# JonasFrey96/Visual-Odom-Pipeline

Hardware: AMD Instinct MI355X
Metric: frames/sec @1241x376, 2000 KLT pts, 10-frame BA window (higher is better)
Workload: dtype u8/i32 (KLT, Shi-Tomasi) + f64 (DLT, BA); 1 GPU; kitti_shaped_1241x376_2000pts_ba10; sequences_per_gpu=256, batched_contexts_per_gpu=1, distinct_image_sequences=8, tracked_points=jittered grid (SURVEY 8d's fallback), launch=plain, solves_stopped_by_cap=0, solves_cut_and_rerun=0

## Files before the change

include/vo_mi355x.h:

```cpp
#ifndef VO_MI355X_H
#define VO_MI355X_H

#include <stdint.h>

#ifdef __cplusplus
extern "C" {
#endif

#define VO_ABI_VERSION 4

enum {
  VO_OK = 0,
  VO_E_INVALID = -1,
  VO_E_HIP = -2,
  VO_E_NOMEM = -3,
  VO_E_STATE = -4,
  VO_E_CAPACITY = -5,
  VO_E_NUMERIC = -6
};

typedef struct vo_ctx vo_ctx;


typedef struct {
// ... 78 lines not shown
  int32_t pad;
} vo_ess_stats;

typedef struct {
  float   x, y;
  float   size;
  float   angle;
  float   response;
  int32_t octave;
} vo_sift_kp;

int32_t vo_abi_version(void);
int32_t vo_device_count(int32_t* n);
int32_t vo_ctx_create(int32_t device, int32_t width, int32_t height, int32_t max_pts,
                      int32_t max_level, int32_t win, vo_ctx** out);
int32_t vo_ctx_create_batched(int32_t device, int32_t width, int32_t height, int32_t max_pts,
                              int32_t max_level, int32_t win, int32_t batch, vo_ctx** out);
int32_t vo_ctx_destroy(vo_ctx* ctx);
const char* vo_last_error(const vo_ctx* ctx);
int32_t vo_sync(vo_ctx* ctx);

int32_t vo_frame_push(vo_ctx* ctx, const uint8_t* img, int32_t stride);
int32_t vo_set_prefilter(vo_ctx* ctx, int32_t d, double sigma_color, double sigma_space);
int32_t vo_set_undistort(vo_ctx* ctx, const double K[4], const double* dist, int32_t n_dist, const double* newK);
int32_t vo_clear_undistort(vo_ctx* ctx);
int32_t vo_get_undistort(vo_ctx* ctx, int32_t* on, double K[4], double dist[8], double newK[4]);
int32_t vo_undistort(vo_ctx* ctx, const uint8_t* img, int32_t stride, uint8_t* out);
int32_t vo_undistort_map_read(vo_ctx* ctx, int16_t* sxy, uint16_t* frac, uint8_t* outside);
int32_t vo_seq_upload(vo_ctx* ctx, const uint8_t* frames, int32_t n_frames);
int32_t vo_frame_push_resident(vo_ctx* ctx, int32_t frame_index);
int32_t vo_pyramid_level_size(vo_ctx* ctx, int32_t level, int32_t* w, int32_t* h);
int32_t vo_pyramid_read(vo_ctx* ctx, int32_t which, int32_t level, uint8_t* img_out, int16_t* deriv_out);
int32_t vo_pyramid_read_seq(vo_ctx* ctx, int32_t seq, int32_t which, int32_t level, uint8_t* img_out, int16_t* deriv_out);

int32_t vo_klt_default_params(vo_klt_params* p);
int32_t vo_klt_track(vo_ctx* ctx, const float* p0, int32_t n, const vo_klt_params* prm,
                     float* p1, uint8_t* status, float* err, int32_t* iters);
int32_t vo_points_upload(vo_ctx* ctx, const float* p, int32_t n);
int32_t vo_points_download(vo_ctx* ctx, float* p, uint8_t* status, float* err, int32_t* iters, int32_t n);
int32_t vo_klt_track_resident(vo_ctx* ctx, int32_t n, const vo_klt_params* prm);

int32_t vo_klt_track_fb(vo_ctx* ctx, const float* p0, int32_t n, const vo_klt_params* prm, float* p1, uint8_t* status, float* err,
                        float* p0r, float* fb_err, int32_t* iters);
int32_t vo_set_fb_check(vo_ctx* ctx, float max_err);
int32_t vo_get_fb_check(vo_ctx* ctx, float* max_err);
int32_t vo_fb_read(vo_ctx* ctx, uint8_t* ok, float* fb_err, int32_t n);

enum { VO_KLT_PREDICT_OFF = 0, VO_KLT_PREDICT_CONST_VELOCITY = 1 };
int32_t vo_klt_track_init(vo_ctx* ctx, const float* p0, const float* guess, int32_t n, const vo_klt_params* prm,
                          float* p1, uint8_t* status, float* err, int32_t* iters);
int32_t vo_klt_track_fb_init(vo_ctx* ctx, const float* p0, const float* guess, int32_t n, const vo_klt_params* prm, float* p1, uint8_t* status,
                             float* err, float* p0r, float* fb_err, int32_t* iters);
int32_t vo_set_klt_predict(vo_ctx* ctx, int32_t mode);
int32_t vo_get_klt_predict(vo_ctx* ctx, int32_t* mode);
int32_t vo_klt_guess_read(vo_ctx* ctx, float* guess, int32_t n);

int32_t vo_st_default_params(vo_st_params* p);
int32_t vo_shi_tomasi(vo_ctx* ctx, const float* cur_pts, int32_t n_cur, int32_t mask_radius,
                      const uint8_t* mask, const vo_st_params* prm, float* out_pts, int32_t* n_out);
int32_t vo_shi_tomasi_resident(vo_ctx* ctx, int32_t n_cur, int32_t mask_radius,
                               const vo_st_params* prm);
int32_t vo_shi_tomasi_fetch(vo_ctx* ctx, float* out_pts, int32_t* n_out);
int32_t vo_shi_tomasi_read(vo_ctx* ctx, float* eig_out, uint8_t* mask_out, int32_t* n_candidates);

typedef struct { int32_t win_x, win_y, zero_x, zero_y, max_count, _pad; double epsilon; } vo_subpix_params;
int32_t vo_subpix_default_params(vo_subpix_params* p);
// ... 177 lines not shown
```

visual-odom-pipeline_amd/csrc/vo_frame.hip:

```cpp
#include "vo_internal.h"

#include <stdlib.h>
#include <string.h>

#include <new>

__device__ __forceinline__ int d_reflect101(int p, int len) {
  if (len == 1) return 0;
  while (p < 0 || p >= len) p = (p < 0) ? -p : 2 * (len - 1) - p;
  return p;
}

struct bil_args {
  int maxk;
  signed char dx[49], dy[49];
  float sw[49];
};

__global__ void __launch_bounds__(256) k_pad_level0_bilateral(const uint8_t* __restrict__ raw, size_t raw_seq_stride,
                                                              const int32_t* __restrict__ frame_idx, int w, int h,
                                                              uint8_t* __restrict__ dst, size_t dst_seq_stride, int pitch,
                                                              int ph, bil_args A, const float* __restrict__ color_w) {
  __shared__ float s_cw[256];
  s_cw[threadIdx.x] = color_w[threadIdx.x];
  __syncthreads();
  const int X = blockIdx.x * blockDim.x + threadIdx.x;
  const int Y = blockIdx.y;
  if (X >= w + 2 * VO_PAD || Y >= ph) return;
  raw += (size_t)blockIdx.z * raw_seq_stride;
  dst += (size_t)blockIdx.z * dst_seq_stride;
  if (frame_idx) raw += (size_t)(*frame_idx) * w * h;
  const int x = d_reflect101(X - VO_PAD, w), y = d_reflect101(Y - VO_PAD, h);
  const int val0 = raw[(size_t)y * w + x];
  float sum = 0.f, wsum = 0.f;
  for (int k = 0; k < A.maxk; k++) {
    const int val = raw[(size_t)d_reflect101(y + A.dy[k], h) * w + d_reflect101(x + A.dx[k], w)];
    const int ad = val > val0 ? val - val0 : val0 - val;
    const float wt = A.sw[k] * s_cw[ad];
    sum += (float)val * wt;
    wsum += wt;
  }
  dst[(size_t)Y * pitch + X] = (uint8_t)(int)__builtin_rintf(sum / wsum);
}
// ... 15 lines not shown

__global__ void __launch_bounds__(256) k_pad_level0(const uint8_t* __restrict__ raw, size_t raw_seq_stride,
                                                    const int32_t* __restrict__ frame_idx, int w, int h,
                                                    uint8_t* __restrict__ dst, size_t dst_seq_stride, int pitch, int ph, int remap) {
  int blk, bseq;
  vo_xcd_assign(blockIdx.z * gridDim.x + blockIdx.x, gridDim.x, remap, blk, bseq);
  const int gpr = (w + 2 * VO_PAD + 15) / 16;
  const unsigned gid = (unsigned)blk * blockDim.x + threadIdx.x;
  const int g_lo = VO_PAD / 16, g_hi = max(g_lo, min(gpr, (w + VO_PAD - 16 >= 0 ? (w + VO_PAD - 16) / 16 + 1 : 0)));
  int Y, G;
  const bool interior = vo_split_index(gid, ph, gpr, g_lo, g_hi, Y, G);
  const int X = G * 16;
  if (Y >= ph) return;
  raw += (size_t)bseq * raw_seq_stride;
  dst += (size_t)bseq * dst_seq_stride;
  if (frame_idx) raw += (size_t)(*frame_idx) * w * h;
  const int y = d_reflect101(Y - VO_PAD, h);
  const uint8_t* row = raw + (size_t)y * w;
  uint32_t v[4];
  if (interior) {
    __builtin_memcpy(v, row + (X - VO_PAD), 16);
  } else {
#pragma unroll
    for (int q = 0; q < 4; q++) {
      v[q] = 0;
#pragma unroll
      for (int k = 0; k < 4; k++) v[q] |= (uint32_t)row[d_reflect101(X + 4 * q + k - VO_PAD, w)] << (8 * k);
    }
  }
  uint4 pk; pk.x = v[0]; pk.y = v[1]; pk.z = v[2]; pk.w = v[3];
  *reinterpret_cast<uint4*>(dst + (size_t)Y * pitch + X) = pk;
}

__device__ __forceinline__ int d_byte(uint32_t v, int k) { return (int)((v >> (8 * k)) & 0xFFu); }

__global__ void __launch_bounds__(256) k_scharr_pyrdown(const uint8_t* __restrict__ src, size_t src_seq_px, int w, int h, int pitch,
                                                        int16_t* __restrict__ der, int nb_scharr,
                                                        uint8_t* __restrict__ dst, size_t dst_seq_px, int dw, int dh, int dpitch, int remap) {
  int bx, bseq;
  vo_xcd_assign(blockIdx.y * gridDim.x + blockIdx.x, gridDim.x, remap, bx, bseq);
  src += (size_t)bseq * src_seq_px;
  if (bx < nb_scharr) {
    constexpr int SR = 4;
    const int gpr = (w + 3) / 4;
    const unsigned gid = (unsigned)bx * 256u + threadIdx.x;
    const int ys = (int)(gid / (unsigned)gpr);
    const int x0 = (int)(gid - (unsigned)ys * (unsigned)gpr) * 4;
    const int y0 = ys * SR;
    if (y0 >= h) return;
    typedef unsigned short u16x2 __attribute__((ext_vector_type(2)));
    typedef short s16x2 __attribute__((ext_vector_type(2)));
    auto load_row = [&](int yy, u16x2 (&a)[3]) {
      const uint32_t* q = reinterpret_cast<const uint32_t*>(src + (size_t)(yy + VO_PAD) * pitch + (x0 + VO_PAD));
      const uint32_t L = q[-1], M = q[0], R = q[1];
      a[0] = __builtin_bit_cast(u16x2, __builtin_amdgcn_perm(M, L, 0x0c040c03u));
      a[1] = __builtin_bit_cast(u16x2, __builtin_amdgcn_perm(0u, M, 0x0c020c01u));
      a[2] = __builtin_bit_cast(u16x2, __builtin_amdgcn_perm(R, M, 0x0c040c03u));
    };
    u16x2 rows[SR + 2][3];
#pragma unroll
    for (int r = 0; r < SR + 2; r++) load_row(min(y0 - 1 + r, h), rows[r]);
#pragma unroll
    for (int r = 0; r < SR; r++) {
      const int y = y0 + r;
      if (y >= h) break;
      s16x2 cs[3], dv[3];
#pragma unroll
      for (int c = 0; c < 3; c++) {
        cs[c] = __builtin_bit_cast(s16x2, (u16x2)((rows[r][c] + rows[r + 2][c]) * (unsigned short)12 + rows[r + 1][c] * (unsigned short)40));
        dv[c] = __builtin_bit_cast(s16x2, (u16x2)(rows[r + 2][c] - rows[r][c]));
      }
      const uint32_t ix01 = __builtin_bit_cast(uint32_t, (s16x2)(cs[1] - cs[0]));
      const uint32_t ix23 = __builtin_bit_cast(uint32_t, (s16x2)(cs[2] - cs[1]));
      const s16x2 w_lo = {12, 40}, w_hi = {40, 12}, w_0 = {12, 0}, w_1 = {0, 12};
      const int iy0 = __builtin_amdgcn_sdot2(dv[1], w_0, __builtin_amdgcn_sdot2(dv[0], w_lo, 0, false), false);
      const int iy1 = __builtin_amdgcn_sdot2(dv[1], w_hi, __builtin_amdgcn_sdot2(dv[0], w_1, 0, false), false);
      const int iy2 = __builtin_amdgcn_sdot2(dv[2], w_0, __builtin_amdgcn_sdot2(dv[1], w_lo, 0, false), false);
      const int iy3 = __builtin_amdgcn_sdot2(dv[2], w_hi, __builtin_amdgcn_sdot2(dv[1], w_1, 0, false), false);
      uint32_t out[4];
      out[0] = __builtin_amdgcn_perm((uint32_t)iy0, ix01, 0x05040100u);
      out[1] = __builtin_amdgcn_perm((uint32_t)iy1, ix01, 0x05040302u);
      out[2] = __builtin_amdgcn_perm((uint32_t)iy2, ix23, 0x05040100u);
      out[3] = __builtin_amdgcn_perm((uint32_t)iy3, ix23, 0x05040302u);
      if (x0 + 3 >= w) {
#pragma unroll
        for (int k = 1; k < 4; k++) if (x0 + k >= w) out[k] = 0u;
      }
      uint4 pk; pk.x = out[0]; pk.y = out[1]; pk.z = out[2]; pk.w = out[3];
      const size_t o = (size_t)(y + VO_PAD) * pitch + (x0 + VO_PAD);
      *reinterpret_cast<uint4*>(reinterpret_cast<uint32_t*>(der) + (size_t)bseq * src_seq_px + o) = pk;
    }
  } else {
    const int b = bx - nb_scharr;
    const int pw = dw + 2 * VO_PAD;
    const int gpr = (pw + 3) / 4;
    const unsigned gid = (unsigned)b * 256u + threadIdx.x;
    const int g_lo = VO_PAD / 4, g_hi = max(g_lo, min(gpr, (dw + VO_PAD - 4 >= 0 ? (dw + VO_PAD - 4) / 4 + 1 : 0)));
    int Y, G;
    const bool interior = vo_split_index(gid, dh + 2 * VO_PAD, gpr, g_lo, g_hi, Y, G);
    const int X0 = G * 4;
    if (Y >= dh + 2 * VO_PAD) return;
    const int y = d_reflect101(Y - VO_PAD, dh);
    const uint8_t* prow = src + (size_t)(2 * y + VO_PAD) * pitch + VO_PAD;
    uint32_t res = 0;
    if (interior) {
      const int x0 = X0 - VO_PAD;
      uint32_t acc[4] = {128u, 128u, 128u, 128u};
#pragma unroll
      for (int j = -2; j <= 2; j++) {
        const uint32_t* q = reinterpret_cast<const uint32_t*>(prow + (ptrdiff_t)j * pitch + 2 * x0);
        const uint32_t d0 = q[-1], d1 = q[0], d2 = q[1], d3 = q[2];
        const uint32_t wj = (j == 0) ? 6u : ((j == -1 || j == 1) ? 4u : 1u);
        acc[0] = __builtin_amdgcn_udot4(d1, wj * 0x00010406u, __builtin_amdgcn_udot4(d0, wj * 0x04010000u, acc[0], false), false);
        acc[1] = __builtin_amdgcn_udot4(d2, wj * 0x00000001u, __builtin_amdgcn_udot4(d1, wj * 0x04060401u, acc[1], false), false);
        acc[2] = __builtin_amdgcn_udot4(d2, wj * 0x00010406u, __builtin_amdgcn_udot4(d1, wj * 0x04010000u, acc[2], false), false);
        acc[3] = __builtin_amdgcn_udot4(d3, wj * 0x00000001u, __builtin_amdgcn_udot4(d2, wj * 0x04060401u, acc[3], false), false);
      }
      res = __builtin_amdgcn_perm(__builtin_amdgcn_perm(acc[3], acc[2], 0x0c0c0501u), __builtin_amdgcn_perm(acc[1], acc[0], 0x0c0c0501u), 0x05040100u);
    } else {
#pragma unroll
      for (int k = 0; k < 4; k++) {
        const int x = d_reflect101(X0 + k - VO_PAD, dw);
        const uint8_t* p = prow + 2 * x;
        int sum = 0;
#pragma unroll
        for (int j = -2; j <= 2; j++) {
          const uint8_t* r = p + (ptrdiff_t)j * pitch;
          const int row = r[-2] + 4 * r[-1] + 6 * r[0] + 4 * r[1] + r[2];
          const int wj = (j == 0) ? 6 : ((j == -1 || j == 1) ? 4 : 1);
          sum += wj * row;
        }
        res |= (uint32_t)((sum + 128) >> 8) << (8 * k);
      }
    }
    *reinterpret_cast<uint32_t*>(dst + (size_t)bseq * dst_seq_px + (size_t)Y * dpitch + X0) = res;
  }
}

static hipEvent_t prof_event(vo_ctx* c) {
  vo_prof& p = c->prof;
  if (p.used == p.pool.size()) {
    hipEvent_t e = nullptr;
    if (hipEventCreate(&e) != hipSuccess) return nullptr;
    p.pool.push_back(e);
  }
  return p.pool[p.used++];
}

vo_prof_scope::vo_prof_scope(vo_ctx* c_, hipStream_t q_, int region_) : c(c_), q(q_), region(region_) {
  if (!((c->prof.mask >> region) & 1)) return;
  e0 = prof_event(c); e1 = prof_event(c);
  if (e0) (void)hipEventRecord(e0, q);
}

vo_prof_scope::~vo_prof_scope() {
  if (!e0 || !e1) return;
  (void)hipEventRecord(e1, q);
  c->prof.pairs[region].push_back(std::make_pair(e0, e1));
}

extern "C" int32_t vo_profile_enable(vo_ctx* c, int32_t region_mask) {
  if (!c) return VO_E_INVALID;
  VO_HIP(c, hipSetDevice(c->device));
  VO_HIP(c, hipStreamSynchronize(c->stream));
  c->prof.mask = region_mask;
  c->prof.used = 0;
  for (int r = 0; r < VO_PROF_COUNT; r++) c->prof.pairs[r].clear();
  return VO_OK;
// ... 189 lines not shown
    CR(hipHostMalloc((void**)&c->h_slab, 2 * c->slab_bytes, hipHostMallocDefault));
  }
  CR(hipMalloc((void**)&c->d_iters, sizeof(int32_t) * (size_t)max_pts * VO_MAX_LEVELS * batch));
  CR(hipMalloc((void**)&c->d_uv0, sizeof(float) * 2 * (size_t)max_pts * batch));
  CR(hipMalloc((void**)&c->d_uv1, sizeof(float) * 2 * (size_t)max_pts * batch));
  CR(hipMalloc((void**)&c->d_frame_idx, sizeof(int32_t)));
  CR(hipHostMalloc((void**)&c->h_frame_idx, sizeof(int32_t) * 64, hipHostMallocDefault));
  CR(hipStreamSynchronize(c->stream));
#undef CR
  *out = c;
  return VO_OK;
}

extern "C" int32_t vo_sync(vo_ctx* c) {
  if (!c) return VO_E_INVALID;
  VO_HIP(c, hipSetDevice(c->device));
  VO_HIP(c, hipStreamSynchronize(c->stream));
  if (c->stream2) VO_HIP(c, hipStreamSynchronize(c->stream2));
  if (c->stream3) VO_HIP(c, hipStreamSynchronize(c->stream3));
  if (c->stream_h2d) VO_HIP(c, hipStreamSynchronize(c->stream_h2d));
  return VO_OK;
}

int32_t vo_build_pyramid(vo_ctx* c, hipStream_t q, const uint8_t* d_raw_img, size_t raw_seq_stride, const int32_t* d_frame_idx) {
  vo_prof_scope prof(c, q, VO_PROF_FRAME);
  c->cur ^= 1;
  vo_frame& F = c->fr[c->cur];
  const int B = c->batch;
  const int remap = (!c->tune.xcd_remap_off && B % 8 == 0) ? 1 : 0;
  if (c->und_on) {
    vo_undistort_enqueue(c, q, d_raw_img, raw_seq_stride, d_frame_idx, remap);
    d_raw_img = c->d_und; raw_seq_stride = (size_t)c->width * c->height; d_frame_idx = nullptr;
  }
  {
    const vo_level& L = c->lv[0];
    dim3 grid(vo_div_up(((L.w + 2 * VO_PAD + 15) / 16) * L.ph, 256), 1, B);
    dim3 grid1(vo_div_up(L.w + 2 * VO_PAD, 256), L.ph, B);
    if (c->bil_maxk > 0) {
      bil_args A;
      A.maxk = c->bil_maxk;
      for (int k = 0; k < 49; k++) { A.dx[k] = c->bil_dx[k]; A.dy[k] = c->bil_dy[k]; A.sw[k] = c->bil_sw[k]; }
      hipLaunchKernelGGL(k_pad_level0_bilateral, grid1, dim3(256), 0, q, d_raw_img, raw_seq_stride, d_frame_idx, L.w,
                         L.h, F.img[0], c->lvl_px[0], L.pitch, L.ph, A, c->d_bil_cw);
    } else {
      hipLaunchKernelGGL(k_pad_level0, grid, dim3(256), 0, q, d_raw_img, raw_seq_stride, d_frame_idx, L.w, L.h,
                         F.img[0], c->lvl_px[0], L.pitch, L.ph, remap);
    }
  }
  for (int l = 0; l <= c->top; l++) {
    const vo_level& L = c->lv[l];
    const int nb_scharr = vo_div_up(vo_div_up(L.w, 4) * vo_div_up(L.h, 4), 256);
    int nb_down = 0;
    uint8_t* dst = nullptr; int dw = 0, dh = 0, dpitch = 0; size_t dpx = 0;
    if (l < c->top) {
      const vo_level& D = c->lv[l + 1];
      dst = F.img[l + 1]; dw = D.w; dh = D.h; dpitch = D.pitch; dpx = c->lvl_px[l + 1];
      nb_down = vo_div_up(vo_div_up(D.w + 2 * VO_PAD, 4) * D.ph, 256);
    }
    hipLaunchKernelGGL(k_scharr_pyrdown, dim3(nb_scharr + nb_down, B), dim3(256), 0, q,
                       F.img[l], c->lvl_px[l], L.w, L.h, L.pitch, F.der[l], nb_scharr, dst, dpx, dw, dh, dpitch, remap);
  }
  VO_HIP(c, hipGetLastError());
  c->n_pushed++;
  return VO_OK;
}

extern "C" int32_t vo_frame_push(vo_ctx* c, const uint8_t* img, int32_t stride) {
  if (!c) return VO_E_INVALID;
  VO_CHECK(c, img != nullptr && stride >= c->width, VO_E_INVALID, "bad image / stride");
  VO_HIP(c, hipSetDevice(c->device));
  { const int32_t rq = vo_quiesce_side(c); if (rq != VO_OK) return rq; }
  const size_t rows = (size_t)c->height * c->batch, bytes = rows * c->width;
  if (!c->h_raw) {
    VO_HIP(c, hipHostMalloc((void**)&c->h_raw, bytes, hipHostMallocDefault));
    VO_HIP(c, hipEventCreateWithFlags(&c->ev_raw, hipEventDisableTiming));
  } else {
    VO_HIP(c, hipEventSynchronize(c->ev_raw));
  }
  if (stride == c->width) memcpy(c->h_raw, img, bytes);
  else for (size_t y = 0; y < rows; y++) memcpy(c->h_raw + y * c->width, img + y * (size_t)stride, c->width);
  VO_HIP(c, hipMemcpyAsync(c->d_raw, c->h_raw, bytes, hipMemcpyHostToDevice, c->stream));
  VO_HIP(c, hipEventRecord(c->ev_raw, c->stream));
  return vo_build_pyramid(c, c->stream, c->d_raw, (size_t)c->width * c->height, nullptr);
}
// ... 22 lines not shown
  return vo_build_pyramid(c, c->stream, c->d_seq + (size_t)idx * fr, fr * c->seq_n, nullptr);
}

extern "C" int32_t vo_pyramid_level_size(vo_ctx* c, int32_t level, int32_t* w, int32_t* h) {
  if (!c) return VO_E_INVALID;
  VO_CHECK(c, level >= 0 && level <= c->top && w && h, VO_E_INVALID, "bad level");
  *w = c->lv[level].w; *h = c->lv[level].h;
  return VO_OK;
}

extern "C" int32_t vo_pyramid_read(vo_ctx* c, int32_t which, int32_t level, uint8_t* img_out, int16_t* deriv_out) {
  return vo_pyramid_read_seq(c, 0, which, level, img_out, deriv_out);
}

extern "C" int32_t vo_pyramid_read_seq(vo_ctx* c, int32_t seq, int32_t which, int32_t level, uint8_t* img_out, int16_t* deriv_out) {
  if (!c) return VO_E_INVALID;
  VO_CHECK(c, level >= 0 && level <= c->top && (which == 0 || which == 1) && seq >= 0 && seq < c->batch, VO_E_INVALID, "bad level / which / seq");
  VO_CHECK(c, c->n_pushed >= (which == 0 ? 2 : 1), VO_E_STATE, "frame not pushed yet");
  VO_HIP(c, hipSetDevice(c->device));
  const vo_frame& F = c->fr[which == 1 ? c->cur : (c->cur ^ 1)];
  const vo_level& L = c->lv[level];
  VO_HIP(c, hipStreamSynchronize(c->stream));
  if (img_out)
    VO_HIP(c, hipMemcpy2D(img_out, L.w, F.img[level] + (size_t)seq * c->lvl_px[level] + (size_t)VO_PAD * L.pitch + VO_PAD, L.pitch, L.w, L.h,
                          hipMemcpyDeviceToHost));
  if (deriv_out)
    VO_HIP(c, hipMemcpy2D(deriv_out, (size_t)L.w * 4, F.der[level] + ((size_t)seq * c->lvl_px[level] + (size_t)VO_PAD * L.pitch + VO_PAD) * 2,
                          (size_t)L.pitch * 4, (size_t)L.w * 4, L.h, hipMemcpyDeviceToHost));
  if (deriv_out)
    for (size_t i = 0, n = (size_t)L.w * L.h * 2; i < n; i++) deriv_out[i] = (int16_t)(deriv_out[i] / 4);
  return VO_OK;
}

extern "C" int32_t vo_set_prefilter(vo_ctx* c, int32_t d, double sigma_color, double sigma_space) {
  if (!c) return VO_E_INVALID;
  if (d == 0) { c->bil_maxk = 0; return VO_OK; }
  if (sigma_color <= 0) sigma_color = 1;
  if (sigma_space <= 0) sigma_space = 1;
  int radius = d < 0 ? (int)lrint(sigma_space * 1.5) : d / 2;
  if (radius < 1) radius = 1;
  VO_CHECK(c, radius <= 3, VO_E_CAPACITY, "bilateral pre-filter: diameter up to 7");
  VO_HIP(c, hipSetDevice(c->device));
  const double gc = -0.5 / (sigma_color * sigma_color), gs = -0.5 / (sigma_space * sigma_space);
  float cw[256];
  for (int i = 0; i < 256; i++) cw[i] = (float)exp((double)i * i * gc);
  int maxk = 0;
  for (int i = -radius; i <= radius; i++)
    for (int j = -radius; j <= radius; j++) {
      const double r = sqrt((double)i * i + (double)j * j);
      if (r > radius) continue;
      c->bil_sw[maxk] = (float)exp(r * r * gs);
      c->bil_dx[maxk] = (signed char)j; c->bil_dy[maxk] = (signed char)i;
      maxk++;
    }
  if (!c->d_bil_cw) VO_HIP(c, hipMalloc((void**)&c->d_bil_cw, sizeof(cw)));
  VO_HIP(c, hipMemcpyAsync(c->d_bil_cw, cw, sizeof(cw), hipMemcpyHostToDevice, c->stream));
  VO_HIP(c, hipStreamSynchronize(c->stream));
  c->bil_maxk = maxk;
  return VO_OK;
}
```

visual-odom-pipeline_amd/vo_mi355x/_lib.py:

```python
import ctypes as C
import os

import numpy as np

_HERE = os.path.dirname(os.path.abspath(__file__))
PKG_ROOT = os.path.dirname(_HERE)
LIB_PATH = os.environ.get("VO_MI355X_LIB") or os.path.join(PKG_ROOT, "lib", "libvo_mi355x.so")
CSRC_DIR = os.path.join(PKG_ROOT, "csrc")

VO_OK = 0
ERRORS = {-1: "VO_E_INVALID", -2: "VO_E_HIP", -3: "VO_E_NOMEM", -4: "VO_E_STATE", -5: "VO_E_CAPACITY",
          -6: "VO_E_NUMERIC"}


class VoError(RuntimeError):
    def __init__(self, code, msg):
        super().__init__("%s (%d): %s" % (ERRORS.get(code, "VO_E_?"), code, msg))
        self.code = code


class KltParams(C.Structure):
    _fields_ = [("win", C.c_int32), ("max_level", C.c_int32), ("max_count", C.c_int32),
                ("epsilon", C.c_double), ("min_eig_threshold", C.c_float), ("_pad", C.c_int32)]

# ... 57 lines not shown
                ("octave", C.c_int32)]


class BaStats(C.Structure):
    _fields_ = [("cost0", C.c_double), ("cost", C.c_double), ("lam", C.c_double), ("iters", C.c_int32),
                ("accepted", C.c_int32), ("status", C.c_int32), ("n_obs", C.c_int32)]


class PipeParams(C.Structure):
    _fields_ = [("ba_window", C.c_int32), ("min_track_length", C.c_int32), ("mask_radius", C.c_int32), ("max_new", C.c_int32),
                ("pnp_blind_batches", C.c_int32), ("ba_budget", C.c_int32), ("resurrect", C.c_int32), ("reserved", C.c_int32),
                ("max_reproj_err", C.c_double),
                ("min_bearing_angle", C.c_double), ("klt", KltParams), ("st", StParams), ("ba", BaParams), ("pnp", PnpParams)]


class PipeRecord(C.Structure):
    _fields_ = [(n, C.c_int32) for n in ("t", "status", "overflow", "n_landmarks", "n_candidates", "n_dead", "n_dead_total", "n_tracked",
                                         "pnp_inliers", "pnp_hypotheses", "pnp_bound_reached", "n_ripe", "n_new", "n_resurrected",
                                         "n_detected", "ba_landmarks", "ba_observations", "ba_iters", "ba_accepted", "ba_status", "ba_done",
                                         "t_final")] + [("ba_cost0", C.c_double), ("ba_cost", C.c_double), ("H", C.c_double * 12),
                                                        ("H_final", C.c_double * 12)]


_u8p, _i16p, _i32p = C.POINTER(C.c_uint8), C.POINTER(C.c_int16), C.POINTER(C.c_int32)
_f32p, _f64p = C.POINTER(C.c_float), C.POINTER(C.c_double)
_ctx = C.c_void_p

SIGNATURES = {
    "vo_abi_version": (C.c_int32, []),
    "vo_device_count": (C.c_int32, [_i32p]),
    "vo_ctx_create": (C.c_int32, [C.c_int32] * 6 + [C.POINTER(_ctx)]),
    "vo_ctx_create_batched": (C.c_int32, [C.c_int32] * 7 + [C.POINTER(_ctx)]),
    "vo_pyramid_read_seq": (C.c_int32, [_ctx, C.c_int32, C.c_int32, C.c_int32, _u8p, _i16p]),
    "vo_ctx_destroy": (C.c_int32, [_ctx]),
    "vo_last_error": (C.c_char_p, [_ctx]),
    "vo_sync": (C.c_int32, [_ctx]),
    "vo_frame_push": (C.c_int32, [_ctx, _u8p, C.c_int32]),
    "vo_set_prefilter": (C.c_int32, [_ctx, C.c_int32, C.c_double, C.c_double]),
    "vo_set_undistort": (C.c_int32, [_ctx, _f64p, _f64p, C.c_int32, _f64p]),
    "vo_clear_undistort": (C.c_int32, [_ctx]),
    "vo_get_undistort": (C.c_int32, [_ctx, _i32p, _f64p, _f64p, _f64p]),
    "vo_undistort": (C.c_int32, [_ctx, _u8p, C.c_int32, _u8p]),
    "vo_undistort_map_read": (C.c_int32, [_ctx, _i16p, C.POINTER(C.c_uint16), _u8p]),
    "vo_seq_upload": (C.c_int32, [_ctx, _u8p, C.c_int32]),
    "vo_frame_push_resident": (C.c_int32, [_ctx, C.c_int32]),
    "vo_pyramid_level_size": (C.c_int32, [_ctx, C.c_int32, _i32p, _i32p]),
    "vo_pyramid_read": (C.c_int32, [_ctx, C.c_int32, C.c_int32, _u8p, _i16p]),
    "vo_klt_default_params": (C.c_int32, [C.POINTER(KltParams)]),
    "vo_klt_track": (C.c_int32, [_ctx, _f32p, C.c_int32, C.POINTER(KltParams), _f32p, _u8p, _f32p, _i32p]),
    "vo_points_upload": (C.c_int32, [_ctx, _f32p, C.c_int32]),
    "vo_points_download": (C.c_int32, [_ctx, _f32p, _u8p, _f32p, _i32p, C.c_int32]),
    "vo_klt_track_resident": (C.c_int32, [_ctx, C.c_int32, C.POINTER(KltParams)]),
    "vo_klt_track_fb": (C.c_int32, [_ctx, _f32p, C.c_int32, C.POINTER(KltParams), _f32p, _u8p, _f32p, _f32p, _f32p, _i32p]),
    "vo_set_fb_check": (C.c_int32, [_ctx, C.c_float]),
    "vo_get_fb_check": (C.c_int32, [_ctx, _f32p]),
    "vo_fb_read": (C.c_int32, [_ctx, _u8p, _f32p, C.c_int32]),
    "vo_klt_track_init": (C.c_int32, [_ctx, _f32p, _f32p, C.c_int32, C.POINTER(KltParams), _f32p, _u8p, _f32p, _i32p]),
    "vo_klt_track_fb_init": (C.c_int32, [_ctx, _f32p, _f32p, C.c_int32, C.POINTER(KltParams), _f32p, _u8p, _f32p, _f32p, _f32p, _i32p]),
    "vo_set_klt_predict": (C.c_int32, [_ctx, C.c_int32]),
    "vo_get_klt_predict": (C.c_int32, [_ctx, _i32p]),
    "vo_klt_guess_read": (C.c_int32, [_ctx, _f32p, C.c_int32]),
    "vo_subpix_default_params": (C.c_int32, [C.POINTER(SubpixParams)]),
    "vo_corner_subpix": (C.c_int32, [_ctx, C.c_int32, _f32p, C.c_int32, C.POINTER(SubpixParams), _f32p, _i32p, _u8p]),
    "vo_set_subpix": (C.c_int32, [_ctx, C.POINTER(SubpixParams)]),
    "vo_get_subpix": (C.c_int32, [_ctx, _i32p, C.POINTER(SubpixParams)]),
    "vo_subpix_read": (C.c_int32, [_ctx, _f32p, _i32p, _u8p, C.c_int32]),
# ... 105 lines not shown
```

visual-odom-pipeline_amd/vo_mi355x/context.py:

```python
import ctypes as C

import numpy as np

from . import _lib
from ._lib import BaParams, BaStats, EssParams, EssStats, KltParams, SiftKp, PnpParams, PnpStats, StParams, SubpixParams, Tuning, VoError, as_c, ptr

KLT_PREDICT_MODES = {"off": 0, "constant_velocity": 1}


class VoContext:
    default_tuning = {}

    def __init__(self, width, height, max_pts=4096, device=0, max_level=3, win=31, batch=1):
        self._L = _lib.load()
        self._h = C.c_void_p()
        rc = self._L.vo_ctx_create_batched(device, width, height, max_pts, max_level, win, batch, C.byref(self._h))
        if rc != 0:
            msg = self._L.vo_last_error(None)
            raise VoError(rc, msg.decode() if msg else "vo_ctx_create failed")
        self.width, self.height, self.max_pts = width, height, max_pts
        self.max_level, self.win, self.device, self.batch = max_level, win, device, batch
        self._st_max_corners = 1000
        self._subpix_slots = 1000
        self._klt_levels = max_level + 1
# ... 103 lines not shown
        frac = np.empty((self.height, self.width), np.uint16)
        out = np.empty((self.height, self.width), np.uint8)
        self._ck(self._L.vo_undistort_map_read(self._h, ptr(sxy, C.c_int16), ptr(frac, C.c_uint16), ptr(out, C.c_uint8)))
        return dict(sxy=sxy, frac=frac, outside=out)

    def push_frame(self, img):
        img = np.asarray(img)
        if img.dtype != np.uint8:
            raise ValueError("push_frame: expected uint8")
        img = self._in(img, np.uint8, (self.height, self.width))
        self._ck(self._L.vo_frame_push(self._h, ptr(img, C.c_uint8), self.width))

    def upload_sequence(self, frames):
        frames = np.asarray(frames, np.uint8)
        if frames.ndim == 3 and self.batch == 1:
            frames = frames[None]
        assert frames.ndim == 4 and frames.shape[0] == self.batch and frames.shape[2:] == (self.height, self.width)
        frames = np.ascontiguousarray(frames)
        self._ck(self._L.vo_seq_upload(self._h, ptr(frames, C.c_uint8), frames.shape[1]))

    def push_frame_resident(self, idx):
        self._ck(self._L.vo_frame_push_resident(self._h, int(idx)))

    def level_size(self, level):
        w, h = C.c_int32(), C.c_int32()
        self._ck(self._L.vo_pyramid_level_size(self._h, level, C.byref(w), C.byref(h)))
        return w.value, h.value

    def pyramid_read(self, which, level, seq=0):
        w, h = self.level_size(level)
        img = np.empty((h, w), np.uint8)
        der = np.empty((h, w, 2), np.int16)
        self._ck(self._L.vo_pyramid_read_seq(self._h, seq, which, level, ptr(img, C.c_uint8), ptr(der, C.c_int16)))
        return img, der

    def klt_params(self, win=None, max_level=None, max_count=30, epsilon=0.03, min_eig_threshold=1e-4):
        p = KltParams()
        self._L.vo_klt_default_params(C.byref(p))
        p.win = self.win if win is None else win
        p.max_level = self.max_level if max_level is None else max_level
        p.max_count, p.epsilon, p.min_eig_threshold = max_count, epsilon, min_eig_threshold
        return p

    def _npts(self, p):
        p = np.asarray(p, np.float32)
        if self.batch == 1:
            p = p.reshape(1, -1, 2)
        if p.ndim != 3 or p.shape[0] != self.batch or p.shape[2] != 2:
            raise ValueError("points must have shape [batch, n, 2]")
        return np.ascontiguousarray(p), p.shape[1]

    def _guess(self, init, n):
        if init is None:
            return None, None
        g, ng = self._npts(init)
        if ng != n:
            raise ValueError("init must have the shape of p0")
        return g, ptr(g, C.c_float)

    def klt_track(self, p0, params=None, return_iters=False, init=None):
        p0, n = self._npts(p0)
        B = self.batch
        prm = params if params is not None else self.klt_params()
        p1 = np.zeros((B, n, 2), np.float32)
        st = np.zeros((B, n), np.uint8)
        err = np.zeros((B, n), np.float32)
# ... 596 lines not shown
```

Measured before the change: 46650 frames/s.

## Fuse level-0 pad, Scharr and pyrdown into one kernel reading raw frames

Replaces the separate level-0 padding kernel and the level-0 Scharr/pyrdown launch with one fused kernel. It reads the raw frame directly, writes the padded image and derivatives together, and builds level 1 from the raw image using reflection indexing. The Scharr strip height also goes from 4 to 8 rows, with rolling row registers to cut redundant row loads. A padded pyramid readback API is added for debugging. This removes a launch and a full round trip of level 0 through memory, at the cost of more complex border handling and possible register pressure.

Result: slower. 45620 frames/s (-2.2%).

```diff
diff --git a/include/vo_mi355x.h b/include/vo_mi355x.h
--- a/include/vo_mi355x.h
+++ b/include/vo_mi355x.h
@@ -134,6 +134,7 @@
 int32_t vo_pyramid_level_size(vo_ctx* ctx, int32_t level, int32_t* w, int32_t* h);
 int32_t vo_pyramid_read(vo_ctx* ctx, int32_t which, int32_t level, uint8_t* img_out, int16_t* deriv_out);
 int32_t vo_pyramid_read_seq(vo_ctx* ctx, int32_t seq, int32_t which, int32_t level, uint8_t* img_out, int16_t* deriv_out);
+int32_t vo_pyramid_read_padded(vo_ctx* ctx, int32_t seq, int32_t which, int32_t level, uint8_t* img_out, int16_t* deriv_out, int32_t* pitch, int32_t* rows);
 
 int32_t vo_klt_default_params(vo_klt_params* p);
 int32_t vo_klt_track(vo_ctx* ctx, const float* p0, int32_t n, const vo_klt_params* prm,
diff --git a/visual-odom-pipeline_amd/csrc/vo_frame.hip b/visual-odom-pipeline_amd/csrc/vo_frame.hip
--- a/visual-odom-pipeline_amd/csrc/vo_frame.hip
+++ b/visual-odom-pipeline_amd/csrc/vo_frame.hip
@@ -9,6 +9,11 @@
   if (len == 1) return 0;
   while (p < 0 || p >= len) p = (p < 0) ? -p : 2 * (len - 1) - p;
   return p;
+}
+
+__device__ __forceinline__ int d_reflect1(int p, int len) {
+  p = p < 0 ? -p : p;
+  return p >= len ? 2 * (len - 1) - p : p;
 }
 
 struct bil_args {
@@ -90,7 +95,165 @@
   *reinterpret_cast<uint4*>(dst + (size_t)Y * pitch + X) = pk;
 }
 
-__device__ __forceinline__ int d_byte(uint32_t v, int k) { return (int)((v >> (8 * k)) & 0xFFu); }
+#ifndef VO_PYR_SR
+#define VO_PYR_SR 8
+#endif
+#ifndef VO_PYR_NT
+#define VO_PYR_NT 0
+#endif
+
+typedef unsigned short u16x2 __attribute__((ext_vector_type(2)));
+typedef short s16x2 __attribute__((ext_vector_type(2)));
+typedef uint32_t u32x4 __attribute__((ext_vector_type(4)));
+
+struct scharr_row { u16x2 a[3]; };
+
+__device__ __forceinline__ scharr_row d_scharr_unpack(uint32_t L, uint32_t M, uint32_t R) {
+  scharr_row r;
+  r.a[0] = __builtin_bit_cast(u16x2, __builtin_amdgcn_perm(M, L, 0x0c040c03u));
+  r.a[1] = __builtin_bit_cast(u16x2, __builtin_amdgcn_perm(0u, M, 0x0c020c01u));
+  r.a[2] = __builtin_bit_cast(u16x2, __builtin_amdgcn_perm(R, M, 0x0c040c03u));
+  return r;
+}
+
+__device__ __forceinline__ u32x4 d_scharr4(const scharr_row& r0, const scharr_row& r1, const scharr_row& r2, int x0, int w) {
+  s16x2 cs[3], dv[3];
+#pragma unroll
+  for (int c = 0; c < 3; c++) {
+    cs[c] = __builtin_bit_cast(s16x2, (u16x2)((r0.a[c] + r2.a[c]) * (unsigned short)12 + r1.a[c] * (unsigned short)40));
+    dv[c] = __builtin_bit_cast(s16x2, (u16x2)(r2.a[c] - r0.a[c]));
+  }
+  const uint32_t ix01 = __builtin_bit_cast(uint32_t, (s16x2)(cs[1] - cs[0]));
+  const uint32_t ix23 = __builtin_bit_cast(uint32_t, (s16x2)(cs[2] - cs[1]));
+  const s16x2 w_lo = {12, 40}, w_hi = {40, 12}, w_0 = {12, 0}, w_1 = {0, 12};
+  const int iy0 = __builtin_amdgcn_sdot2(dv[1], w_0, __builtin_amdgcn_sdot2(dv[0], w_lo, 0, false), false);
+  const int iy1 = __builtin_amdgcn_sdot2(dv[1], w_hi, __builtin_amdgcn_sdot2(dv[0], w_1, 0, false), false);
+  const int iy2 = __builtin_amdgcn_sdot2(dv[2], w_0, __builtin_amdgcn_sdot2(dv[1], w_lo, 0, false), false);
+  const int iy3 = __builtin_amdgcn_sdot2(dv[2], w_hi, __builtin_amdgcn_sdot2(dv[1], w_1, 0, false), false);
+  u32x4 out;
+  out.x = __builtin_amdgcn_perm((uint32_t)iy0, ix01, 0x05040100u);
+  out.y = __builtin_amdgcn_perm((uint32_t)iy1, ix01, 0x05040302u);
+  out.z = __builtin_amdgcn_perm((uint32_t)iy2, ix23, 0x05040100u);
+  out.w = __builtin_amdgcn_perm((uint32_t)iy3, ix23, 0x05040302u);
+  if (x0 + 3 >= w) {
+    if (x0 + 1 >= w) out.y = 0u;
+    if (x0 + 2 >= w) out.z = 0u;
+    out.w = 0u;
+  }
+  return out;
+}
+
+__device__ __forceinline__ void d_store_der(uint32_t* p, u32x4 v) {
+#if VO_PYR_NT
+  __builtin_nontemporal_store(v, reinterpret_cast<u32x4*>(p));
+#else
+  *reinterpret_cast<u32x4*>(p) = v;
+#endif
+}
+
+__device__ __forceinline__ void d_load3_unaligned(const uint8_t* p, uint32_t& L, uint32_t& M, uint32_t& R) {
+  uint32_t v[3];
+  __builtin_memcpy(v, p - 4, 12);
+  L = v[0]; M = v[1]; R = v[2];
+}
+
+template <int SR>
+__device__ __forceinline__ void d_scharr_strip(const uint8_t* __restrict__ src, int w, int h, int pitch, uint32_t* __restrict__ der, unsigned gid) {
+  const int gpr = (w + 3) / 4;
+  const int ys = (int)(gid / (unsigned)gpr);
+  const int x0 = (int)(gid - (unsigned)ys * (unsigned)gpr) * 4;
+  const int y0 = ys * SR;
+  if (y0 >= h) return;
+  auto fetch = [&](int yy, uint32_t& L, uint32_t& M, uint32_t& R) {
+    const uint32_t* q = reinterpret_cast<const uint32_t*>(src + (size_t)(min(yy, h) + VO_PAD) * pitch + (x0 + VO_PAD));
+    L = q[-1]; M = q[0]; R = q[1];
+  };
+  uint32_t L, M, R;
+  fetch(y0 - 1, L, M, R);
+  scharr_row a = d_scharr_unpack(L, M, R);
+  fetch(y0, L, M, R);
+  scharr_row b = d_scharr_unpack(L, M, R);
+  fetch(y0 + 1, L, M, R);
+#pragma unroll
+  for (int r = 0; r < SR; r++) {
+    const int y = y0 + r;
+    const scharr_row c = d_scharr_unpack(L, M, R);
+    if (r + 1 < SR) fetch(y + 2, L, M, R);
+    const u32x4 out = d_scharr4(a, b, c, x0, w);
+    if (y < h) d_store_der(der + (size_t)(y + VO_PAD) * pitch + (x0 + VO_PAD), out);
+    a = b; b = c;
+  }
+}
+
+template <bool RAW>
+__device__ __forceinline__ void d_pyrdown4(const uint8_t* __restrict__ src, int w, int h, int pitch,
+                                           uint8_t* __restrict__ dst, int dw, int dh, int dpitch, unsigned gid) {
+  const int pw = dw + 2 * VO_PAD;
+  const int gpr = (pw + 3) / 4;
+  int g_lo, g_hi;
+  if (RAW) {
+    const int xm = min(dw - 4, (w - 12) >> 1);
+    g_lo = VO_PAD / 4 + 1;
+    g_hi = xm >= 4 ? min(gpr, xm / 4 + VO_PAD / 4 + 1) : g_lo;
+  } else {
+    g_lo = VO_PAD / 4;
+    g_hi = max(g_lo, min(gpr, (dw + VO_PAD - 4 >= 0 ? (dw + VO_PAD - 4) / 4 + 1 : 0)));
+  }
+  int Y, G;
+  const bool interior = vo_split_index(gid, dh + 2 * VO_PAD, gpr, g_lo, g_hi, Y, G);
+  const int X0 = G * 4;
+  if (Y >= dh + 2 * VO_PAD) return;
+  const int y = d_reflect101(Y - VO_PAD, dh);
+  auto tap_row = [&](int j) -> const uint8_t* {
+    if (RAW) return src + (size_t)d_reflect1(2 * y + j, h) * pitch;
+    return src + (size_t)(2 * y + j + VO_PAD) * pitch + VO_PAD;
+  };
+  uint32_t res = 0;
+  if (interior) {
+    const int x0 = X0 - VO_PAD;
+    uint32_t acc[4] = {128u, 128u, 128u, 128u};
+#pragma unroll
+    for (int j = -2; j <= 2; j++) {
+      uint32_t d[4];
+      const uint8_t* p = tap_row(j) + 2 * x0 - 4;
+      if (RAW) {
+        __builtin_memcpy(d, p, 16);
+      } else {
+        const uint32_t* q = reinterpret_cast<const uint32_t*>(p);
+        d[0] = q[0]; d[1] = q[1]; d[2] = q[2]; d[3] = q[3];
+      }
+      const uint32_t wj = (j == 0) ? 6u : ((j == -1 || j == 1) ? 4u : 1u);
+      acc[0] = __builtin_amdgcn_udot4(d[1], wj * 0x00010406u, __builtin_amdgcn_udot4(d[0], wj * 0x04010000u, acc[0], false), false);
+      acc[1] = __builtin_amdgcn_udot4(d[2], wj * 0x00000001u, __builtin_amdgcn_udot4(d[1], wj * 0x04060401u, acc[1], false), false);
+      acc[2] = __builtin_amdgcn_udot4(d[2], wj * 0x00010406u, __builtin_amdgcn_udot4(d[1], wj * 0x04010000u, acc[2], false), false);
+      acc[3] = __builtin_amdgcn_udot4(d[3], wj * 0x00000001u, __builtin_amdgcn_udot4(d[2], wj * 0x04060401u, acc[3], false), false);
+    }
+    res = __builtin_amdgcn_perm(__builtin_amdgcn_perm(acc[3], acc[2], 0x0c0c0501u), __builtin_amdgcn_perm(acc[1], acc[0], 0x0c0c0501u), 0x05040100u);
+  } else {
+    constexpr int UNR = RAW ? 1 : 4;
+#pragma unroll UNR
+    for (int k = 0; k < 4; k++) {
+      const int x = d_reflect101(X0 + k - VO_PAD, dw);
+      int sum = 0;
+#pragma unroll
+      for (int j = -2; j <= 2; j++) {
+        const uint8_t* r = tap_row(j);
+        int row;
+        if (RAW) {
+          row = r[d_reflect1(2 * x - 2, w)] + 4 * r[d_reflect1(2 * x - 1, w)] + 6 * r[2 * x] + 4 * r[d_reflect1(2 * x + 1, w)] +
+                r[d_reflect1(2 * x + 2, w)];
+        } else {
+          r += 2 * x;
+          row = r[-2] + 4 * r[-1] + 6 * r[0] + 4 * r[1] + r[2];
+        }
+        const int wj = (j == 0) ? 6 : ((j == -1 || j == 1) ? 4 : 1);
+        sum += wj * row;
+      }
+      res |= (uint32_t)((sum + 128) >> 8) << (8 * k);
+    }
+  }
+  *reinterpret_cast<uint32_t*>(dst + (size_t)Y * dpitch + X0) = res;
+}
 
 __global__ void __launch_bounds__(256) k_scharr_pyrdown(const uint8_t* __restrict__ src, size_t src_seq_px, int w, int h, int pitch,
                                                         int16_t* __restrict__ der, int nb_scharr,
@@ -99,99 +262,111 @@
   vo_xcd_assign(blockIdx.y * gridDim.x + blockIdx.x, gridDim.x, remap, bx, bseq);
   src += (size_t)bseq * src_seq_px;
   if (bx < nb_scharr) {
-    constexpr int SR = 4;
-    const int gpr = (w + 3) / 4;
+    d_scharr_strip<VO_PYR_SR>(src, w, h, pitch, reinterpret_cast<uint32_t*>(der) + (size_t)bseq * src_seq_px, (unsigned)bx * 256u + threadIdx.x);
+  } else {
+    d_pyrdown4<false>(src, w, h, pitch, dst + (size_t)bseq * dst_seq_px, dw, dh, dpitch, (unsigned)(bx - nb_scharr) * 256u + threadIdx.x);
+  }
+}
+
+#define VO_L0_MIN_W 36
+__global__ void __launch_bounds__(256, 8) k_level0_fused(const uint8_t* __restrict__ raw, size_t raw_seq_stride, const int32_t* __restrict__ frame_idx,
+                                                      int w, int h, uint8_t* __restrict__ img, size_t seq_px, int pitch, int16_t* __restrict__ der,
+                                                      int nb_int, int nb_down,
+                                                      uint8_t* __restrict__ dst, size_t dst_seq_px, int dw, int dh, int dpitch, int remap) {
+  constexpr int SR = VO_PYR_SR;
+  int bx, bseq;
+  vo_xcd_assign(blockIdx.y * gridDim.x + blockIdx.x, gridDim.x, remap, bx, bseq);
+  raw += (size_t)bseq * raw_seq_stride;
+  if (frame_idx) raw += (size_t)(*frame_idx) * w * h;
+  img += (size_t)bseq * seq_px;
+  uint32_t* der32 = reinterpret_cast<uint32_t*>(der) + (size_t)bseq * seq_px;
+  const int x_hi = ((w - 4) / 16) * 16;
+  if (bx < nb_int) {
+    const int gi = (x_hi - 16) / 4;
     const unsigned gid = (unsigned)bx * 256u + threadIdx.x;
-    const int ys = (int)(gid / (unsigned)gpr);
-    const int x0 = (int)(gid - (unsigned)ys * (unsigned)gpr) * 4;
+    const int ys = (int)(gid / (unsigned)gi);
+    const int x0 = 16 + (int)(gid - (unsigned)ys * (unsigned)gi) * 4;
     const int y0 = ys * SR;
     if (y0 >= h) return;
-    typedef unsigned short u16x2 __attribute__((ext_vector_type(2)));
-    typedef short s16x2 __attribute__((ext_vector_type(2)));
-    auto load_row = [&](int yy, u16x2 (&a)[3]) {
-      const uint32_t* q = reinterpret_cast<const uint32_t*>(src + (size_t)(yy + VO_PAD) * pitch + (x0 + VO_PAD));
-      const uint32_t L = q[-1], M = q[0], R = q[1];
-      a[0] = __builtin_bit_cast(u16x2, __builtin_amdgcn_perm(M, L, 0x0c040c03u));
-      a[1] = __builtin_bit_cast(u16x2, __builtin_amdgcn_perm(0u, M, 0x0c020c01u));
-      a[2] = __builtin_bit_cast(u16x2, __builtin_amdgcn_perm(R, M, 0x0c040c03u));
+    auto fetch = [&](int yy, uint32_t& L, uint32_t& M, uint32_t& R) {
+      d_load3_unaligned(raw + (size_t)d_reflect1(min(yy, h), h) * w + x0, L, M, R);
     };
-    u16x2 rows[SR + 2][3];
-#pragma unroll
-    for (int r = 0; r < SR + 2; r++) load_row(min(y0 - 1 + r, h), rows[r]);
+    uint32_t L, M, R;
+    fetch(y0 - 1, L, M, R);
+    scharr_row a = d_scharr_unpack(L, M, R);
+    fetch(y0, L, M, R);
+    scharr_row b = d_scharr_unpack(L, M, R);
+    uint32_t mb = M;
+    fetch(y0 + 1, L, M, R);
 #pragma unroll
     for (int r = 0; r < SR; r++) {
       const int y = y0 + r;
-      if (y >= h) break;
-      s16x2 cs[3], dv[3];
-#pragma unroll
-      for (int c = 0; c < 3; c++) {
-        cs[c] = __builtin_bit_cast(s16x2, (u16x2)((rows[r][c] + rows[r + 2][c]) * (unsigned short)12 + rows[r + 1][c] * (unsigned short)40));
-        dv[c] = __builtin_bit_cast(s16x2, (u16x2)(rows[r + 2][c] - rows[r][c]));
+      const scharr_row c = d_scharr_unpack(L, M, R);
+      const uint32_t mc = M;
+      if (r + 1 < SR) fetch(y + 2, L, M, R);
+      const u32x4 out = d_scharr4(a, b, c, x0, w);
+      if (y < h) {
+        const size_t o = (size_t)(y + VO_PAD) * pitch + (x0 + VO_PAD);
+        *reinterpret_cast<uint32_t*>(img + o) = mb;
+        d_store_der(der32 + o, out);
       }
-      const uint32_t ix01 = __builtin_bit_cast(uint32_t, (s16x2)(cs[1] - cs[0]));
-      const uint32_t ix23 = __builtin_bit_cast(uint32_t, (s16x2)(cs[2] - cs[1]));
-      const s16x2 w_lo = {12, 40}, w_hi = {40, 12}, w_0 = {12, 0}, w_1 = {0, 12};
-      const int iy0 = __builtin_amdgcn_sdot2(dv[1], w_0, __builtin_amdgcn_sdot2(dv[0], w_lo, 0, false), false);
-      const int iy1 = __builtin_amdgcn_sdot2(dv[1], w_hi, __builtin_amdgcn_sdot2(dv[0], w_1, 0, false), false);
-      const int iy2 = __builtin_amdgcn_sdot2(dv[2], w_0, __builtin_amdgcn_sdot2(dv[1], w_lo, 0, false), false);
-      const int iy3 = __builtin_amdgcn_sdot2(dv[2], w_hi, __builtin_amdgcn_sdot2(dv[1], w_1, 0, false), false);
-      uint32_t out[4];
-      out[0] = __builtin_amdgcn_perm((uint32_t)iy0, ix01, 0x05040100u);
-      out[1] = __builtin_amdgcn_perm((uint32_t)iy1, ix01, 0x05040302u);
-      out[2] = __builtin_amdgcn_perm((uint32_t)iy2, ix23, 0x05040100u);
-      out[3] = __builtin_amdgcn_perm((uint32_t)iy3, ix23, 0x05040302u);
-      if (x0 + 3 >= w) {
-#pragma unroll
-        for (int k = 1; k < 4; k++) if (x0 + k >= w) out[k] = 0u;
+      a = b; b = c; mb = mc;
+    }
+  } else if (bx < nb_int + nb_down) {
+    d_pyrdown4<true>(raw, w, h, w, dst + (size_t)bseq * dst_seq_px, dw, dh, dpitch, (unsigned)(bx - nb_int) * 256u + threadIdx.x);
+  } else {
+    const int ph = h + 2 * VO_PAD;
+    const int gpr = (w + 2 * VO_PAD + 15) / 16;
+    const int g_lo = (16 + VO_PAD) / 16, g_hi = (x_hi + VO_PAD) / 16;
+    const int gi = g_hi - g_lo, gb = gpr - gi;
+    const int ne = 4 + (w - x_hi + 3) / 4;
+    const unsigned n1 = (unsigned)(2 * VO_PAD) * (unsigned)gi, n2 = (unsigned)ph * (unsigned)gb, n3 = (unsigned)h * (unsigned)ne;
+    unsigned id = (unsigned)(bx - nb_int - nb_down) * 256u + threadIdx.x;
+    if (id < n1 + n2) {
+      int Y, G;
+      const bool copy = id < n1;
+      if (copy) {
+        const int r = (int)(id / (unsigned)gi);
+        G = g_lo + (int)(id - (unsigned)r * (unsigned)gi);
+        Y = r < VO_PAD ? r : h + r;
+      } else {
+        id -= n1;
+        Y = (int)(id / (unsigned)gb);
+        const int j = (int)(id - (unsigned)Y * (unsigned)gb);
+        G = j < g_lo ? j : g_hi + (j - g_lo);
       }
-      uint4 pk; pk.x = out[0]; pk.y = out[1]; pk.z = out[2]; pk.w = out[3];
-      const size_t o = (size_t)(y + VO_PAD) * pitch + (x0 + VO_PAD);
-      *reinterpret_cast<uint4*>(reinterpret_cast<uint32_t*>(der) + (size_t)bseq * src_seq_px + o) = pk;
-    }
-  } else {
-    const int b = bx - nb_scharr;
-    const int pw = dw + 2 * VO_PAD;
-    const int gpr = (pw + 3) / 4;
-    const unsigned gid = (unsigned)b * 256u + threadIdx.x;
-    const int g_lo = VO_PAD / 4, g_hi = max(g_lo, min(gpr, (dw + VO_PAD - 4 >= 0 ? (dw + VO_PAD - 4) / 4 + 1 : 0)));
-    int Y, G;
-    const bool interior = vo_split_index(gid, dh + 2 * VO_PAD, gpr, g_lo, g_hi, Y, G);
-    const int X0 = G * 4;
-    if (Y >= dh + 2 * VO_PAD) return;
-    const int y = d_reflect101(Y - VO_PAD, dh);
-    const uint8_t* prow = src + (size_t)(2 * y + VO_PAD) * pitch + VO_PAD;
-    uint32_t res = 0;
-    if (interior) {
-      const int x0 = X0 - VO_PAD;
-      uint32_t acc[4] = {128u, 128u, 128u, 128u};
-#pragma unroll
-      for (int j = -2; j <= 2; j++) {
-        const uint32_t* q = reinterpret_cast<const uint32_t*>(prow + (ptrdiff_t)j * pitch + 2 * x0);
-        const uint32_t d0 = q[-1], d1 = q[0], d2 = q[1], d3 = q[2];
-        const uint32_t wj = (j == 0) ? 6u : ((j == -1 || j == 1) ? 4u : 1u);
-        acc[0] = __builtin_amdgcn_udot4(d1, wj * 0x00010406u, __builtin_amdgcn_udot4(d0, wj * 0x04010000u, acc[0], false), false);
-        acc[1] = __builtin_amdgcn_udot4(d2, wj * 0x00000001u, __builtin_amdgcn_udot4(d1, wj * 0x04060401u, acc[1], false), false);
-        acc[2] = __builtin_amdgcn_udot4(d2, wj * 0x00010406u, __builtin_amdgcn_udot4(d1, wj * 0x04010000u, acc[2], false), false);
-        acc[3] = __builtin_amdgcn_udot4(d3, wj * 0x00000001u, __builtin_amdgcn_udot4(d2, wj * 0x04060401u, acc[3], false), false);
+      const int X = G * 16;
+      const uint8_t* row = raw + (size_t)d_reflect101(Y - VO_PAD, h) * w;
+      uint32_t v[4];
+      if (copy) {
+        __builtin_memcpy(v, row + (X - VO_PAD), 16);
+      } else {
+#pragma unroll
+        for (int q = 0; q < 4; q++) {
+          v[q] = 0;
+#pragma unroll
+          for (int k = 0; k < 4; k++) v[q] |= (uint32_t)row[d_reflect101(X + 4 * q + k - VO_PAD, w)] << (8 * k);
+        }
       }
-      res = __builtin_amdgcn_perm(__builtin_amdgcn_perm(acc[3], acc[2], 0x0c0c0501u), __builtin_amdgcn_perm(acc[1], acc[0], 0x0c0c0501u), 0x05040100u);
-    } else {
-#pragma unroll
-      for (int k = 0; k < 4; k++) {
-        const int x = d_reflect101(X0 + k - VO_PAD, dw);
-        const uint8_t* p = prow + 2 * x;
-        int sum = 0;
-#pragma unroll
-        for (int j = -2; j <= 2; j++) {
-          const uint8_t* r = p + (ptrdiff_t)j * pitch;
-          const int row = r[-2] + 4 * r[-1] + 6 * r[0] + 4 * r[1] + r[2];
-          const int wj = (j == 0) ? 6 : ((j == -1 || j == 1) ? 4 : 1);
-          sum += wj * row;
-        }
-        res |= (uint32_t)((sum + 128) >> 8) << (8 * k);
+      uint4 pk; pk.x = v[0]; pk.y = v[1]; pk.z = v[2]; pk.w = v[3];
+      *reinterpret_cast<uint4*>(img + (size_t)Y * pitch + X) = pk;
+    } else if (id - (n1 + n2) < n3) {
+      id -= n1 + n2;
+      const int y = (int)(id / (unsigned)ne);
+      const int j = (int)(id - (unsigned)y * (unsigned)ne);
+      const int x0 = j < 4 ? 4 * j : x_hi + 4 * (j - 4);
+      int col[6];
+#pragma unroll
+      for (int k = 0; k < 6; k++) col[k] = d_reflect1(x0 - 1 + k, w);
+      scharr_row rw[3];
+#pragma unroll
+      for (int r = 0; r < 3; r++) {
+        const uint8_t* row = raw + (size_t)d_reflect1(y - 1 + r, h) * w;
+#pragma unroll
+        for (int k = 0; k < 3; k++) { rw[r].a[k].x = row[col[2 * k]]; rw[r].a[k].y = row[col[2 * k + 1]]; }
       }
-    }
-    *reinterpret_cast<uint32_t*>(dst + (size_t)bseq * dst_seq_px + (size_t)Y * dpitch + X0) = res;
+      d_store_der(der32 + (size_t)(y + VO_PAD) * pitch + (x0 + VO_PAD), d_scharr4(rw[0], rw[1], rw[2], x0, w));
+    }
   }
 }
 
@@ -447,24 +622,38 @@
     vo_undistort_enqueue(c, q, d_raw_img, raw_seq_stride, d_frame_idx, remap);
     d_raw_img = c->d_und; raw_seq_stride = (size_t)c->width * c->height; d_frame_idx = nullptr;
   }
-  {
-    const vo_level& L = c->lv[0];
-    dim3 grid(vo_div_up(((L.w + 2 * VO_PAD + 15) / 16) * L.ph, 256), 1, B);
-    dim3 grid1(vo_div_up(L.w + 2 * VO_PAD, 256), L.ph, B);
-    if (c->bil_maxk > 0) {
-      bil_args A;
-      A.maxk = c->bil_maxk;
-      for (int k = 0; k < 49; k++) { A.dx[k] = c->bil_dx[k]; A.dy[k] = c->bil_dy[k]; A.sw[k] = c->bil_sw[k]; }
-      hipLaunchKernelGGL(k_pad_level0_bilateral, grid1, dim3(256), 0, q, d_raw_img, raw_seq_stride, d_frame_idx, L.w,
-                         L.h, F.img[0], c->lvl_px[0], L.pitch, L.ph, A, c->d_bil_cw);
-    } else {
-      hipLaunchKernelGGL(k_pad_level0, grid, dim3(256), 0, q, d_raw_img, raw_seq_stride, d_frame_idx, L.w, L.h,
-                         F.img[0], c->lvl_px[0], L.pitch, L.ph, remap);
-    }
-  }
-  for (int l = 0; l <= c->top; l++) {
+  const vo_level& L0 = c->lv[0];
+  int first = 0;
+  if (c->bil_maxk > 0) {
+    dim3 grid1(vo_div_up(L0.w + 2 * VO_PAD, 256), L0.ph, B);
+    bil_args A;
+    A.maxk = c->bil_maxk;
+    for (int k = 0; k < 49; k++) { A.dx[k] = c->bil_dx[k]; A.dy[k] = c->bil_dy[k]; A.sw[k] = c->bil_sw[k]; }
+    hipLaunchKernelGGL(k_pad_level0_bilateral, grid1, dim3(256), 0, q, d_raw_img, raw_seq_stride, d_frame_idx, L0.w,
+                       L0.h, F.img[0], c->lvl_px[0], L0.pitch, L0.ph, A, c->d_bil_cw);
+  } else if (L0.w < VO_L0_MIN_W) {
+    dim3 grid(vo_div_up(((L0.w + 2 * VO_PAD + 15) / 16) * L0.ph, 256), 1, B);
+    hipLaunchKernelGGL(k_pad_level0, grid, dim3(256), 0, q, d_raw_img, raw_seq_stride, d_frame_idx, L0.w, L0.h,
+                       F.img[0], c->lvl_px[0], L0.pitch, L0.ph, remap);
+  } else {
+    const int x_hi = ((L0.w - 4) / 16) * 16;
+    const int nb_int = vo_div_up(((x_hi - 16) / 4) * vo_div_up(L0.h, VO_PYR_SR), 256);
+    const int gb = (L0.w + 2 * VO_PAD + 15) / 16 - (x_hi - 16) / 16;
+    const int nb_rest = vo_div_up(2 * VO_PAD * ((x_hi - 16) / 16) + L0.ph * gb + L0.h * (4 + (L0.w - x_hi + 3) / 4), 256);
+    int nb_down = 0;
+    uint8_t* dst = nullptr; int dw = 0, dh = 0, dpitch = 0; size_t dpx = 0;
+    if (c->top > 0) {
+      const vo_level& D = c->lv[1];
+      dst = F.img[1]; dw = D.w; dh = D.h; dpitch = D.pitch; dpx = c->lvl_px[1];
+      nb_down = vo_div_up(vo_div_up(D.w + 2 * VO_PAD, 4) * D.ph, 256);
+    }
+    hipLaunchKernelGGL(k_level0_fused, dim3(nb_int + nb_down + nb_rest, B), dim3(256), 0, q, d_raw_img, raw_seq_stride, d_frame_idx, L0.w, L0.h,
+                       F.img[0], c->lvl_px[0], L0.pitch, F.der[0], nb_int, nb_down, dst, dpx, dw, dh, dpitch, remap);
+    first = 1;
+  }
+  for (int l = first; l <= c->top; l++) {
     const vo_level& L = c->lv[l];
-    const int nb_scharr = vo_div_up(vo_div_up(L.w, 4) * vo_div_up(L.h, 4), 256);
+    const int nb_scharr = vo_div_up(vo_div_up(L.w, 4) * vo_div_up(L.h, VO_PYR_SR), 256);
     int nb_down = 0;
     uint8_t* dst = nullptr; int dw = 0, dh = 0, dpitch = 0; size_t dpx = 0;
     if (l < c->top) {
@@ -553,6 +742,24 @@
   return VO_OK;
 }
 
+extern "C" int32_t vo_pyramid_read_padded(vo_ctx* c, int32_t seq, int32_t which, int32_t level, uint8_t* img_out, int16_t* deriv_out, int32_t* pitch,
+                                          int32_t* rows) {
+  if (!c) return VO_E_INVALID;
+  VO_CHECK(c, level >= 0 && level <= c->top && (which == 0 || which == 1) && seq >= 0 && seq < c->batch, VO_E_INVALID, "bad level / which / seq");
+  const vo_level& L = c->lv[level];
+  if (pitch) *pitch = L.pitch;
+  if (rows) *rows = L.ph;
+  if (!img_out && !deriv_out) return VO_OK;
+  VO_CHECK(c, c->n_pushed >= (which == 0 ? 2 : 1), VO_E_STATE, "frame not pushed yet");
+  VO_HIP(c, hipSetDevice(c->device));
+  const vo_frame& F = c->fr[which == 1 ? c->cur : (c->cur ^ 1)];
+  VO_HIP(c, hipStreamSynchronize(c->stream));
+  const size_t px = c->lvl_px[level];
+  if (img_out) VO_HIP(c, hipMemcpy(img_out, F.img[level] + (size_t)seq * px, px, hipMemcpyDeviceToHost));
+  if (deriv_out) VO_HIP(c, hipMemcpy(deriv_out, F.der[level] + (size_t)seq * px * 2, px * 4, hipMemcpyDeviceToHost));
+  return VO_OK;
+}
+
 extern "C" int32_t vo_set_prefilter(vo_ctx* c, int32_t d, double sigma_color, double sigma_space) {
   if (!c) return VO_E_INVALID;
   if (d == 0) { c->bil_maxk = 0; return VO_OK; }
diff --git a/visual-odom-pipeline_amd/vo_mi355x/_lib.py b/visual-odom-pipeline_amd/vo_mi355x/_lib.py
--- a/visual-odom-pipeline_amd/vo_mi355x/_lib.py
+++ b/visual-odom-pipeline_amd/vo_mi355x/_lib.py
@@ -113,6 +113,7 @@
     "vo_ctx_create": (C.c_int32, [C.c_int32] * 6 + [C.POINTER(_ctx)]),
     "vo_ctx_create_batched": (C.c_int32, [C.c_int32] * 7 + [C.POINTER(_ctx)]),
     "vo_pyramid_read_seq": (C.c_int32, [_ctx, C.c_int32, C.c_int32, C.c_int32, _u8p, _i16p]),
+    "vo_pyramid_read_padded": (C.c_int32, [_ctx, C.c_int32, C.c_int32, C.c_int32, _u8p, _i16p, _i32p, _i32p]),
     "vo_ctx_destroy": (C.c_int32, [_ctx]),
     "vo_last_error": (C.c_char_p, [_ctx]),
     "vo_sync": (C.c_int32, [_ctx]),
diff --git a/visual-odom-pipeline_amd/vo_mi355x/context.py b/visual-odom-pipeline_amd/vo_mi355x/context.py
--- a/visual-odom-pipeline_amd/vo_mi355x/context.py
+++ b/visual-odom-pipeline_amd/vo_mi355x/context.py
@@ -159,6 +159,14 @@
         img = np.empty((h, w), np.uint8)
         der = np.empty((h, w, 2), np.int16)
         self._ck(self._L.vo_pyramid_read_seq(self._h, seq, which, level, ptr(img, C.c_uint8), ptr(der, C.c_int16)))
+        return img, der
+
+    def pyramid_read_padded(self, which, level, seq=0):
+        pitch, rows = C.c_int32(), C.c_int32()
+        self._ck(self._L.vo_pyramid_read_padded(self._h, seq, which, level, None, None, C.byref(pitch), C.byref(rows)))
+        img = np.empty((rows.value, pitch.value), np.uint8)
+        der = np.empty((rows.value, pitch.value, 2), np.int16)
+        self._ck(self._L.vo_pyramid_read_padded(self._h, seq, which, level, ptr(img, C.c_uint8), ptr(der, C.c_int16), None, None))
         return img, der
 
     def klt_params(self, win=None, max_level=None, max_count=30, epsilon=0.03, min_eig_threshold=1e-4):
```
